# jim-ec/constraint_solver

Hardware: AMD Instinct MI355X
Metric: body·substeps/sec at 262k rigid bodies, 20 substeps/frame; 1/2/4/8 GPU (higher is better)
Workload: dtype f64

## Files before the change

### constraint_solver_amd/csrc/xpbd_contacts.h

```cpp
#pragma once

#include "xpbd_pairs.h"

namespace xpbd {

struct Joint {
    uint32_t body_a, body_b;
    double anchor_a[3], anchor_b[3];
    double distance;
    double axis_a[3], axis_b[3];
    uint32_t kind, reserved;
};

struct JointLimit {
    uint32_t joint, kind;
    double ref_a[3], ref_b[3];
    double lower, upper;
};

struct GridInfo {
    double edge;
    int32_t origin[3];
    uint32_t dims[3];
    uint32_t dense;
// ... 20 lines not shown
    uint32_t *nbr_pair;
    uint32_t *pairs;
    double *rec;
    const double *stat_rec;
    const uint32_t *stat_index;
    ContactManifold *manifolds;
    uint8_t *pair_codes;
    unsigned long long *stats;
    uint32_t *scan_scratch;
    const Joint *joints;
    const uint32_t *joint_off;
    const uint32_t *joint_list;
    const JointLimit *limits;
    const uint32_t *limit_off;
    double max_depenetration_speed;
    const uint2 *filter;
    uint32_t *slot_filter;
    uint32_t filter_jointed;
    const double *friction;
    double ground_friction;
    const double *restitution;
    double ground_restitution;
    double bounce_threshold;
};

struct BodySubset {
    const uint32_t *list = nullptr;
    uint32_t count = 0;
    const uint8_t *skip = nullptr;
    double *export_rows = nullptr;
    const double *import_buf = nullptr;
    const uint32_t *import_rows = nullptr;
};

hipError_t launch_bounds_and_cells(const BodyArrays &b, const PolytopeTables &t, const double *shape_radius,
                                   double dt, double pad, const ContactBuffers &c, hipStream_t stream);
hipError_t launch_build_buckets(const BodyArrays &b, const ContactBuffers &c, hipStream_t stream);
hipError_t launch_neighbour_count(const BodyArrays &b, const ContactBuffers &c, hipStream_t stream);
hipError_t launch_neighbour_fill(const BodyArrays &b, const ContactBuffers &c, hipStream_t stream);

hipError_t launch_integrate_ground(const BodyArrays &b, const ShapeTable &s, double h, const ContactBuffers &c,
                                   uint32_t *last_mask, uint32_t *trace_masks, uint32_t trace_row, hipStream_t stream,
                                   const BodySubset &subset = BodySubset());
hipError_t launch_sat_contact_pairs(const BodyArrays &b, const PolytopeTables &t, const ContactBuffers &c,
                                    uint32_t n_pairs, SatScratch *list, hipStream_t stream, bool dense = false);
hipError_t launch_pair_solve_derive(const BodyArrays &b, double *dyn_out, double h, const ContactBuffers &c,
                                    hipStream_t stream, const BodySubset &subset = BodySubset());

hipError_t launch_pair_solve_integrate_ground(const BodyArrays &b, const ShapeTable &s, double h, const ContactBuffers &c,
                                              double *next_rec, uint32_t *last_mask, uint32_t *trace_masks, uint32_t trace_row,
                                              hipStream_t stream, const BodySubset &subset = BodySubset());

hipError_t launch_restitution(const BodyArrays &b, const double *post, const double *start, const ShapeTable &s, const ContactBuffers &c,
                              const uint32_t *ground_masks, hipStream_t stream);

hipError_t launch_body_frames(const BodyArrays &b, double *rec, hipStream_t stream);
hipError_t launch_stat_records(const BodyArrays &b, double *stat_rec, hipStream_t stream);
hipError_t launch_body_frames_aos(const BodyArrays &b, double *frames, hipStream_t stream);

hipError_t launch_export_dynamic(const BodyArrays &b, const uint32_t *indices, uint32_t n, double *buf, hipStream_t stream);
hipError_t launch_import_dynamic(const BodyArrays &b, const uint32_t *indices, const uint32_t *rows, uint32_t n, const double *buf,
                                 hipStream_t stream);

constexpr uint32_t kMaxEditEntries = 1u << 29;
hipError_t launch_set_wrench(const BodyArrays &b, const uint32_t *indices, uint32_t n, const double *force, const double *torque,
                             hipStream_t stream);
hipError_t launch_apply_impulses(const BodyArrays &b, const xpbd_impulse *list, uint32_t n, hipStream_t stream);

// ... 13 lines not shown
```

### constraint_solver_amd/csrc/xpbd_contacts.hip

```cpp
#include <cfloat>
#include <type_traits>

#include "xpbd_contacts.h"
#include "xpbd_step.hpp"

namespace xpbd {
namespace {

constexpr uint32_t kBlock = 256;
#ifndef XPBD_SMALL_WORLD
#define XPBD_SMALL_WORLD 16384
#endif
constexpr uint32_t kSmallWorld = XPBD_SMALL_WORLD;
#ifndef XPBD_PAIR_SOLVE_MIN_WAVES
#define XPBD_PAIR_SOLVE_MIN_WAVES 2
#endif

__device__ __forceinline__ uint32_t cell_hash(int32_t x, int32_t y, int32_t z)
{
    return ((uint32_t)x * 73856093u) ^ ((uint32_t)y * 19349663u) ^ ((uint32_t)z * 83492791u);
}

__device__ __forceinline__ uint32_t block_scan_exclusive(uint32_t v, uint32_t *total)
{
    __shared__ uint32_t wave_sum[kBlock / 64];
    const uint32_t lane = threadIdx.x & 63u, wave = threadIdx.x >> 6;
    uint32_t inc = v;
#pragma unroll
    for (uint32_t d = 1; d < 64; d <<= 1) {
        const uint32_t up = __shfl_up(inc, d, 64);
        if (lane >= d)
            inc += up;
    }
    if (lane == 63)
        wave_sum[wave] = inc;
    __syncthreads();
    uint32_t before = 0, all = 0;
#pragma unroll
// ... 604 lines not shown
    p.pos = r.pos;
    p.rot = r.rot;
    p.inv_mass = s.inv_mass;
    p.inv_inertia = s.inv_inertia;
    p.com = s.com;
    p.p1 = r.p1;
    p.past = r.past;
    if (past_pos)
        *past_pos = r.past_pos;
    return p;
}

__device__ __forceinline__ Vec3 frame_delta(const Frame &cur, const Frame &past, Vec3 global)
{
    const Vec3 local = inverse(cur) * global;
    return global - past * local;
}

template <class Body>
__device__ __forceinline__ double generalized_inverse_mass(const Body &p, Vec3 point, Vec3 dir)
{
    const Vec3 angular_impulse = conjugate(p.rot) * cross(point - (p.pos + p.com), dir);
    return p.inv_mass + dot(p.inv_inertia * angular_impulse, angular_impulse);
}

#ifndef XPBD_JOINT_LIMIT_INLINE
#define XPBD_JOINT_LIMIT_INLINE __forceinline__
#endif
__device__ XPBD_JOINT_LIMIT_INLINE void joint_limit_terms(const ContactBuffers &c, uint32_t joint, const Joint &jt, bool self_is_a,
                                                          const PairBody &self, const PairBody &other, double compliance, Quat &drot,
                                                          uint32_t &count)
{
    const uint32_t l_end = c.limit_off[joint + 1];
    for (uint32_t l = c.limit_off[joint]; l < l_end; ++l) {
        const JointLimit &lim = c.limits[l];
        const Quat q_a = self_is_a ? self.rot : other.rot, q_b = self_is_a ? other.rot : self.rot;
        const Vec3 a_w = q_a * Vec3{jt.axis_a[0], jt.axis_a[1], jt.axis_a[2]};
        double phi;
        Vec3 n;
        if (lim.kind == XPBD_LIMIT_SWING) {
            const Vec3 b_w = q_b * Vec3{jt.axis_b[0], jt.axis_b[1], jt.axis_b[2]};
            const Vec3 cr = cross(a_w, b_w);
            const double s = length(cr);
            if (s == 0.0)
                continue;
            phi = atan2(s, dot(a_w, b_w));
// ... 12 lines not shown
                p_a = p_a - n * dot(p_a, n);
                p_b = p_b - n * dot(p_b, n);
            }
            phi = atan2(dot(cross(p_a, p_b), n), dot(p_a, p_b));
        }
        const double clamped = phi < lim.lower ? lim.lower : (phi > lim.upper ? lim.upper : phi);
        const double err = phi - clamped;
        if (err == 0.0)
            continue;
        const Vec3 n_self = conjugate(self.rot) * n, n_other = conjugate(other.rot) * n;
        const double w_s = dot(self.inv_inertia * n_self, n_self), w_o = dot(other.inv_inertia * n_other, n_other);
        const double w = self_is_a ? w_s + w_o : w_o + w_s;
        const double lambda = err / (w + compliance);
        const Vec3 turn = self_is_a ? lambda * n : (-lambda) * n;
        const Quat spin = quat_sv(0.0, self.inv_inertia * turn);
        drot = drot + (0.5 * spin) * self.rot;
        ++count;
    }
}

#ifndef XPBD_PAIR_SOLVE_ROUND_POINTS
#define XPBD_PAIR_SOLVE_ROUND_POINTS 2
#endif
template <uint32_t G, bool MATERIALS>
__device__ __forceinline__ BodyDynamic pair_solve_derive_body(const ContactBuffers &c, uint32_t i, double h,
                                                              const PairBody &self, Vec3 self_past_pos, uint32_t sub, uint32_t &touching,
                                                              uint32_t &points, const RecordStage &stage = RecordStage())
{
    static_assert(G == 1 || G == kMaxManifoldPoints, "one lane per body or one lane per manifold point");
    const double compliance = 1e-6 / (h * h);
    const double limit = c.max_depenetration_speed > 0.0 ? c.max_depenetration_speed * h : 0.0;
    const double mu_self = MATERIALS ? c.friction[i] : 0.0;

    Vec3 dpos{0.0, 0.0, 0.0};
    Quat drot{0.0, 0.0, 0.0, 0.0};
    uint32_t count = 0;
    auto neighbour_terms = [&](uint32_t j, const ContactManifold *m, uint32_t n_points, uint32_t feature, uint32_t pt_begin, uint32_t pt_end) {
        if (j > i && pt_begin == 0) {
            ++touching;
            points += n_points;
        }
        const PairBody other = load_pair_body(c, j, nullptr, stage);
        const double mu = MATERIALS ? min_mu(mu_self, c.friction[j]) : 0.0;
        const bool self_is_a = i < j;
        const bool ref_is_a = feature != 1u;
        const bool self_is_inc = self_is_a != ref_is_a;
        const bool face = feature != 2u;
        const Plane ref_plane{Vec3{m->plane[0], m->plane[1], m->plane[2]}, m->plane[3]};
        auto point_term = [&](uint32_t pt, Vec3 &term_pos, Quat &term_rot) {
            const Vec3 p_inc{m->point[pt][0], m->point[pt][1], m->point[pt][2]};
            Vec3 p_ref;
            if (face) {
                const double depth = distance(ref_plane, p_inc);
                p_ref = p_inc - depth * ref_plane.normal;
            } else {
                p_ref = Vec3{m->point[1][0], m->point[1][1], m->point[1][2]};
            }
            const Vec3 p_self = self_is_inc ? p_inc : p_ref, p_other = self_is_inc ? p_ref : p_inc;
            const Vec3 correction = p_ref - p_inc;
            const Vec3 moved_self = frame_delta(self.p1, self.past, p_self), moved_other = frame_delta(other.p1, other.past, p_other);
            const Vec3 delta_rel = self_is_inc ? moved_self - moved_other : moved_other - moved_self;
            const Vec3 delta_tangential = delta_rel - project_on(delta_rel, correction);
            const Vec3 c0 = p_inc;
// ... 70 lines not shown
                    touch |= 1ull << (k0 - k_base + u);
        }
        uint32_t j_next = 0, pair_next = 0;
        if (touch) {
            const uint32_t k = k_base + (uint32_t)__ffsll((long long)touch) - 1u;
            j_next = c.nbr[k], pair_next = c.nbr_pair[k];
        }
        const uint32_t chunk = (G > 1 || few) ? kMaxManifoldPoints : (uint32_t)XPBD_PAIR_SOLVE_ROUND_POINTS;
        uint32_t j_cur = 0, pair_cur = 0, code_cur = 0, n_cur = 0, pt = 0;
        while (touch || pt < n_cur) {
            if (pt == n_cur) {
                j_cur = j_next, pair_cur = pair_next;
                touch &= touch - 1ull;
                if (touch) {
                    const uint32_t k = k_base + (uint32_t)__ffsll((long long)touch) - 1u;
                    j_next = c.nbr[k], pair_next = c.nbr_pair[k];
                }
                code_cur = c.pair_codes[pair_cur];
                n_cur = code_cur & ((1u << kPairCodeFeatureShift) - 1u);
                pt = 0;
            }
            if (n_cur) {
                const uint32_t stop = n_cur - pt > chunk ? pt + chunk : n_cur;
                neighbour_terms(j_cur, c.manifolds + pair_cur, n_cur, code_cur >> kPairCodeFeatureShift, pt, stop);
                pt = stop;
            }
        }
    }

    if (c.joint_off) {
        for (uint32_t k = c.joint_off[i]; k < c.joint_off[i + 1]; ++k) {
            const Joint &jt = c.joints[c.joint_list[k]];
            const bool self_is_a = jt.body_a == i;
            const PairBody other = load_pair_body(c, self_is_a ? jt.body_b : jt.body_a, nullptr, stage);
            const Vec3 anchor_self = self_is_a ? Vec3{jt.anchor_a[0], jt.anchor_a[1], jt.anchor_a[2]} : Vec3{jt.anchor_b[0], jt.anchor_b[1], jt.anchor_b[2]};
            const Vec3 anchor_other = self_is_a ? Vec3{jt.anchor_b[0], jt.anchor_b[1], jt.anchor_b[2]} : Vec3{jt.anchor_a[0], jt.anchor_a[1], jt.anchor_a[2]};
            const Vec3 p_self = Frame{frame_origin(self.pos, self.rot, self.com), self.rot} * anchor_self;
            const Vec3 p_other = Frame{frame_origin(other.pos, other.rot, other.com), other.rot} * anchor_other;
            const Vec3 difference = self_is_a ? p_other - p_self : p_self - p_other;
            const double dist = length(difference);
            if (dist != 0.0) {
                const Vec3 dir = difference * (1.0 / dist);
                const double w = generalized_inverse_mass(self, p_self, dir) + generalized_inverse_mass(other, p_other, dir);
                const double lambda = (dist - jt.distance) / (w + compliance);
                const Vec3 impulse = self_is_a ? lambda * dir : (-lambda) * dir;
                dpos = dpos + impulse * self.inv_mass;
                const Vec3 arm = p_self - (self.pos + self.com);
// ... 41 lines not shown
    for (uint32_t off = 32; off; off >>= 1) {
        touching += __shfl_xor(touching, off, 64);
        points += __shfl_xor(points, off, 64);
    }
    __shared__ uint32_t part[2][kBlock / 64];
    if ((threadIdx.x & 63u) == 0) {
        part[0][threadIdx.x >> 6] = touching;
        part[1][threadIdx.x >> 6] = points;
    }
    __syncthreads();
    if (threadIdx.x == 0) {
        uint32_t t = 0, p = 0;
        for (uint32_t w = 0; w < kBlock / 64; ++w) {
            t += part[0][w];
            p += part[1][w];
        }
        if (t)
            atomicAdd(&stats[0], (unsigned long long)t);
        if (p)
            atomicAdd(&stats[1], (unsigned long long)p);
    }
}

template <uint32_t G, bool MATERIALS>
__global__ void __launch_bounds__(kBlock, XPBD_PAIR_SOLVE_MIN_WAVES) k_pair_solve_derive(BodyArrays b, double *__restrict__ dyn_out, double h,
                                                                                        ContactBuffers c, BodySubset subset)
{
    const uint32_t gid = blockIdx.x * blockDim.x + threadIdx.x, slot = gid / G, sub = gid % G;
    constexpr bool kStage = G == 1 && XPBD_PAIR_SOLVE_STAGE_RECORDS;
    __shared__ double2 stage_words[kStage ? 12 * kBlock : 1];
    RecordStage stage;
    if (kStage && !subset.list)
        stage = stage_records(stage_words, c.rec, blockIdx.x * kBlock, b.n);
    uint32_t touching = 0, points = 0, i;
    if (subset_body(subset, b.n, slot, i)) {
        Vec3 past_pos;
        const PairBody self = load_pair_body(c, i, &past_pos, stage);
        const BodyDynamic d = pair_solve_derive_body<G, MATERIALS>(c, i, h, self, past_pos, sub, touching, points, stage);
        if (sub == 0) {
            store_dynamic(dyn_out, b.stride, i, d);
            if (subset.export_rows)
                store_row(subset.export_rows, slot, d);
        }
    }
    block_add_stats(sub == 0 ? touching : 0u, sub == 0 ? points : 0u, c.stats);
}

template <bool TRACE, uint32_t G, bool MATERIALS>
__global__ void __launch_bounds__(kBlock, XPBD_PAIR_SOLVE_MIN_WAVES) k_pair_solve_integrate_ground(
    BodyArrays b, ShapeTable shapes, double h, ContactBuffers c, BodySubset subset, double *__restrict__ next_rec,
    uint32_t *__restrict__ last_mask, uint32_t *__restrict__ trace_masks, uint32_t trace_row)
{
    extern __shared__ double lds[];
    uint32_t *lds_off = reinterpret_cast<uint32_t *>(lds + 3 * shapes.total_verts);
    for (uint32_t k = threadIdx.x; k < 3 * shapes.total_verts; k += blockDim.x)
        lds[k] = shapes.verts[k];
    for (uint32_t k = threadIdx.x; k <= shapes.n_shapes; k += blockDim.x)
        lds_off[k] = shapes.offsets[k];
    __syncthreads();

    const uint32_t gid = blockIdx.x * blockDim.x + threadIdx.x, slot = gid / G, sub = gid % G;
    constexpr bool kStage = G == 1 && XPBD_PAIR_SOLVE_STAGE_RECORDS;
    __shared__ double2 stage_words[kStage ? 12 * kBlock : 1];
    RecordStage stage;
    if (kStage && !subset.list)
        stage = stage_records(stage_words, c.rec, blockIdx.x * kBlock, b.n);
    uint32_t touching = 0, points = 0, i;
    if (subset_body(subset, b.n, slot, i)) {
        const uint32_t st = b.stride;
        BodyDynamic d;
        BodyStatic s;
        {
            Vec3 past_pos;
            const PairBody self = load_pair_body(c, i, &past_pos, stage);
            d = pair_solve_derive_body<G, MATERIALS>(c, i, h, self, past_pos, sub, touching, points, stage);
            s = static_of(b, i, self.inv_mass, self.inv_inertia, self.com);
        }
        if (subset.export_rows && sub == 0)
            store_row(subset.export_rows, slot, d);
        const uint32_t sid = b.shape_id[i];
        const uint32_t v0 = lds_off[sid];
        const double compliance = 1e-6 / (h * h);
        const SubstepFrames f = integrate_body(d, s, h);
        const uint32_t mask = solve_ground<MATERIALS>(d, s, f, compliance, lds + 3 * v0, lds_off[sid + 1] - v0,
                                                      c.max_depenetration_speed > 0.0 ? c.max_depenetration_speed * h : 0.0,
                                                      MATERIALS ? ground_mu(c, i) : 0.0);
        if (sub == 0) {
            store_record(next_rec, i, f.cur, f.past, d.pos, d.rot, f.past_pos);
            last_mask[i] = mask;
            if (TRACE)
                trace_masks[(size_t)trace_row * st + i] = mask;
        }
    }
    block_add_stats(sub == 0 ? touching : 0u, sub == 0 ? points : 0u, c.stats);
}

struct VelBody {
    Vec3 pos;
// ... 458 lines not shown
    if (trace_masks && c.friction)
        launch(std::true_type{}, std::true_type{});
    else if (trace_masks)
        launch(std::true_type{}, std::false_type{});
    else if (c.friction)
        launch(std::false_type{}, std::true_type{});
    else
        launch(std::false_type{}, std::false_type{});
    return hipGetLastError();
}

hipError_t launch_sat_contact_pairs(const BodyArrays &b, const PolytopeTables &t, const ContactBuffers &c,
                                    uint32_t n_pairs, SatScratch *list, hipStream_t stream, bool dense)
{
    return launch_sat_contacts(b, t, c.rec, c.pairs, n_pairs, c.manifolds, c.pair_codes, list, stream, dense);
}

hipError_t launch_pair_solve_derive(const BodyArrays &b, double *dyn_out, double h, const ContactBuffers &c,
                                    hipStream_t stream, const BodySubset &subset)
{
    const uint32_t items = subset.list ? subset.count : b.n;
    if (items == 0)
        return hipSuccess;
    auto launch = [&](auto lanes, auto materials) {
        constexpr uint32_t G = decltype(lanes)::value;
        hipLaunchKernelGGL((k_pair_solve_derive<G, decltype(materials)::value>), dim3(blocks_for(items * G)), dim3(kBlock), 0, stream, b,
                           dyn_out, h, c, subset);
    };
    using Wide = std::integral_constant<uint32_t, kMaxManifoldPoints>;
    using One = std::integral_constant<uint32_t, 1>;
    const bool small = b.n <= kSmallWorld;
    if (small && c.friction)
        launch(Wide{}, std::true_type{});
    else if (small)
        launch(Wide{}, std::false_type{});
    else if (c.friction)
        launch(One{}, std::true_type{});
    else
        launch(One{}, std::false_type{});
    return hipGetLastError();
}

hipError_t launch_restitution(const BodyArrays &b, const double *post, const double *start, const ShapeTable &s, const ContactBuffers &c,
                              const uint32_t *ground_masks, hipStream_t stream)
{
    if (b.n == 0)
        return hipSuccess;
    if (!c.restitution || post == b.dyn || start == b.dyn)
        return hipErrorInvalidValue;
    const size_t lds_bytes = (size_t)s.total_verts * 3 * sizeof(double) + (size_t)(s.n_shapes + 1) * sizeof(uint32_t);
    hipLaunchKernelGGL(k_restitution, dim3(blocks_for(b.n)), dim3(kBlock), lds_bytes, stream, b, post, start, s, c, ground_masks);
    return hipGetLastError();
}

hipError_t launch_pair_solve_integrate_ground(const BodyArrays &b, const ShapeTable &s, double h, const ContactBuffers &c,
                                              double *next_rec, uint32_t *last_mask, uint32_t *trace_masks, uint32_t trace_row,
                                              hipStream_t stream, const BodySubset &subset)
{
    const uint32_t items = subset.list ? subset.count : b.n;
    if (items == 0)
        return hipSuccess;
    const size_t lds_bytes = (size_t)s.total_verts * 3 * sizeof(double) + (size_t)(s.n_shapes + 1) * sizeof(uint32_t);
    auto launch_form = [&](auto trace, auto lanes, auto materials) {
        constexpr uint32_t G = decltype(lanes)::value;
        hipLaunchKernelGGL((k_pair_solve_integrate_ground<decltype(trace)::value, G, decltype(materials)::value>), dim3(blocks_for(items * G)),
                           dim3(kBlock), lds_bytes, stream, b, s, h, c, subset, next_rec, last_mask, trace_masks, trace_row);
    };
    auto launch = [&](auto trace, auto lanes) {
        if (c.friction)
            launch_form(trace, lanes, std::true_type{});
        else
            launch_form(trace, lanes, std::false_type{});
    };
    using Wide = std::integral_constant<uint32_t, kMaxManifoldPoints>;
    using One = std::integral_constant<uint32_t, 1>;
    const bool small = b.n <= kSmallWorld;
    if (trace_masks && small)
        launch(std::true_type{}, Wide{});
    else if (trace_masks)
        launch(std::true_type{}, One{});
    else if (small)
        launch(std::false_type{}, Wide{});
    else
        launch(std::false_type{}, One{});
    return hipGetLastError();
}

hipError_t launch_body_frames_aos(const BodyArrays &b, double *frames, hipStream_t stream)
{
    if (b.n)
        hipLaunchKernelGGL(k_body_frames_aos, dim3(blocks_for(b.n)), dim3(kBlock), 0, stream, b, frames);
    return hipGetLastError();
}

hipError_t launch_export_dynamic(const BodyArrays &b, const uint32_t *indices, uint32_t n, double *buf, hipStream_t stream)
{
    if (n)
        hipLaunchKernelGGL(k_export_dynamic, dim3(blocks_for(n * kDynFields)), dim3(kBlock), 0, stream, b, indices, n, buf);
    return hipGetLastError();
}

hipError_t launch_import_dynamic(const BodyArrays &b, const uint32_t *indices, const uint32_t *rows, uint32_t n, const double *buf,
                                 hipStream_t stream)
{
    if (n)
        hipLaunchKernelGGL(k_import_dynamic, dim3(blocks_for(n * kDynFields)), dim3(kBlock), 0, stream, b, indices, rows, n, buf);
    return hipGetLastError();
// ... 78 lines not shown
```

### constraint_solver_amd/csrc/xpbd_world.cpp

```cpp
#include <algorithm>
#include <cmath>
#include <cstdio>
#include <cstdlib>
#include <cstring>
#include <exception>
#include <limits>
#include <memory>
#include <utility>
#include <vector>

#include <hip/hip_runtime_api.h>

#include "xpbd_internal.h"
#include "xpbd_kernels.h"
#include "xpbd_math.hpp"
#include "xpbd_contacts.h"
#include "xpbd_gjk.h"
#include "xpbd_pairs.h"
#include "xpbd_query.h"
#include "xpbd_report.h"

namespace {

uint32_t round_up(uint32_t v, uint32_t to) { return (v + to - 1) / to * to; }
// ... 55 lines not shown
    struct BroadphaseTotals {
        uint32_t entries, pairs;
        unsigned long long stats[2];
    };
    BroadphaseTotals *bp_totals = nullptr;
    hipEvent_t bp_event = nullptr;
    bool bp_pending = false;
    DeviceBuffer frame_snapshot;
    bool frame_snapshot_valid = false, frame_snapshot_stepped = false;
    struct Joints {
        uint32_t n = 0, n_limits = 0;
        std::vector<xpbd_joint> host;
        void clear() { *this = Joints{}; }
    } joints;
    DeviceBuffer jt_joints, jt_off, jt_list, jt_limits, jt_limit_off;
    struct Filters {
        bool on = false;
        uint32_t flags = 0;
        void clear() { *this = Filters{}; }
    } filters;
    DeviceBuffer ft_filters, cb_slot_filter;
    struct Materials {
        bool on = false;
        double ground_friction = std::numeric_limits<double>::infinity();
        void clear() { *this = Materials{}; }
    } materials;
    DeviceBuffer mt_friction;
    struct Restitution {
        bool on = false;
        double ground = 0.0, bounce_threshold = 0.0;
        void clear() { *this = Restitution{}; }
    } restitution;
    DeviceBuffer rs_restitution, rs_start;
    DeviceBuffer q_rec, q_partials, q_grid, q_cell_start, q_cell_fill, q_items, q_scan, q_brute, q_rays, q_hits;
    DeviceBuffer ed_indices, ed_values, ed_list;
    DeviceBuffer history;
    uint32_t history_length = 0;
    std::vector<uint8_t> history_stepped;
    size_t history_slot_bytes() const { return ((size_t)xpbd::kDynFields * stride * 8 + (size_t)stride * 4 + 255) / 256 * 256; }
    DeviceBuffer sat_counters, sat_survivors, sat_axis_cache, gjk_axis_cache, cb_pair_codes;
    xpbd::SatScratch sat_scratch{nullptr, nullptr, 0, nullptr, true};
    bool sat_two_pass = false;
    uint32_t sat_schedule = XPBD_SAT_SCHEDULE_AUTO;
    unsigned long long stats_touching_seen = 0, stats_pair_substeps = 0, stats_pair_substeps_seen = 0;
    DeviceBuffer gjk_counters, gjk_pairs_scratch;
    xpbd::GjkScratch gjk_scratch{nullptr, nullptr, 0, nullptr, nullptr};
    bool report_on = false;
    bool report_frame = false;
    bool report_keys_ready = false;
    bool report_ready = false;
    bool report_prev_valid = false;
    uint32_t report_substeps = 0, report_cur = 0;
    uint32_t report_counts[4] = {0, 0, 0, 0};
    uint32_t *rep_host = nullptr;
    DeviceBuffer rep_touch, rep_flag, rep_sel, rep_npts, rep_keys[2], rep_scan, rep_ev_flag, rep_pairs, rep_points, rep_events;
    const uint8_t *rep_map_owned = nullptr;
    const uint32_t *rep_map_ids = nullptr;
    xpbd::ContactBuffers contact_buffers(uint32_t frame_set = 0) const
    {
        xpbd::ContactBuffers c{};
        c.centers = cb_centers.as<double>();
        c.radius = cb_radius.as<double>();
        c.cell = cb_cell.as<int32_t>();
// ... 14 lines not shown
        c.nbr_pair = cb_nbr_pair.as<uint32_t>();
        c.pairs = cb_pairs.as<uint32_t>();
        c.rec = (frame_set ? cb_rec_b : cb_rec).as<double>();
        c.stat_rec = stat_shared ? cb_stat_shape.as<double>() : cb_stat_rec.as<double>();
        c.stat_index = stat_shared ? shape_id.as<uint32_t>() : nullptr;
        c.manifolds = cb_manifolds.as<xpbd::ContactManifold>();
        c.pair_codes = cb_pair_codes.as<uint8_t>();
        c.stats = cb_stats.as<unsigned long long>();
        c.scan_scratch = cb_scan.as<uint32_t>();
        c.joints = joints.n ? jt_joints.as<xpbd::Joint>() : nullptr;
        c.joint_off = joints.n ? jt_off.as<uint32_t>() : nullptr;
        c.joint_list = joints.n ? jt_list.as<uint32_t>() : nullptr;
        c.limits = joints.n_limits ? jt_limits.as<xpbd::JointLimit>() : nullptr;
        c.limit_off = joints.n_limits ? jt_limit_off.as<uint32_t>() : nullptr;
        c.filter = filters.on ? ft_filters.as<uint2>() : nullptr;
        c.slot_filter = filters.on ? cb_slot_filter.as<uint32_t>() : nullptr;
        c.filter_jointed = (filters.flags & XPBD_FILTER_JOINTED) ? 1u : 0u;
        c.max_depenetration_speed = max_depenetration_speed;
        c.friction = materials.on ? mt_friction.as<double>() : nullptr;
        c.ground_friction = materials.ground_friction;
        c.restitution = restitution.on ? rs_restitution.as<double>() : nullptr;
        c.ground_restitution = restitution.ground;
        c.bounce_threshold = restitution.bounce_threshold;
        return c;
    }

    xpbd::BodyArrays arrays() const
    {
        return xpbd::BodyArrays{dyn.as<double>(), stat.as<double>(), shape_id.as<uint32_t>(), stride, n};
    }
    xpbd::ShapeTable shapes() const
    {
        return xpbd::ShapeTable{shape_verts.as<double>(), shape_offsets.as<uint32_t>(), n_shapes, total_verts};
    }

    ~xpbd_world()
    {
        (void)hipSetDevice(device);
        if (stream)
            (void)hipStreamSynchronize(stream);
        if (bp_totals)
            (void)hipHostFree(bp_totals);
        if (bp_event)
            (void)hipEventDestroy(bp_event);
        if (rep_host)
            (void)hipHostFree(rep_host);
// ... 217 lines not shown
        w->stats_touching_seen = stats_now[0];
        w->stats_pair_substeps_seen = w->stats_pair_substeps;
    }
    if (!w->sat_counters.ptr) {
        XPBD_HIP_TRY(w->sat_counters.reserve(2 * xpbd::kSurvivorCounters * 4));
        XPBD_HIP_TRY(hipMemsetAsync(w->sat_counters.ptr, 0, 2 * xpbd::kSurvivorCounters * 4, w->stream));
        w->sat_scratch.calls = 0;
    }
    XPBD_HIP_TRY(w->sat_survivors.reserve((size_t)(w->n_pairs ? w->n_pairs : 1) * 2 * 4));
    XPBD_HIP_TRY(w->sat_axis_cache.reserve((size_t)(w->n_pairs ? w->n_pairs : 1) * 2));
    XPBD_HIP_TRY(hipMemsetAsync(w->sat_axis_cache.ptr, 0, (size_t)(w->n_pairs ? w->n_pairs : 1) * 2, w->stream));
    w->sat_scratch.counters = w->sat_counters.as<uint32_t>();
    w->sat_scratch.survivors = w->sat_survivors.as<uint32_t>();
    w->sat_scratch.axis_cache = w->sat_axis_cache.as<uint16_t>();
    if (w->narrowphase == XPBD_NARROWPHASE_GJK_EPA) {
        XPBD_HIP_TRY(w->gjk_axis_cache.reserve((size_t)(w->n_pairs ? w->n_pairs : 1) * 24));
        XPBD_HIP_TRY(hipMemsetAsync(w->gjk_axis_cache.ptr, 0, (size_t)(w->n_pairs ? w->n_pairs : 1) * 24, w->stream));
    }
    XPBD_HIP_TRY(w->cb_nbr.reserve((size_t)(w->n_entries ? w->n_entries : 1) * 4));
    XPBD_HIP_TRY(w->cb_nbr_pair.reserve((size_t)(w->n_entries ? w->n_entries : 1) * 4));
    XPBD_HIP_TRY(w->cb_pairs.reserve((size_t)(w->n_pairs ? w->n_pairs : 1) * 8));
    XPBD_HIP_TRY(w->cb_manifolds.reserve((size_t)(w->n_pairs ? w->n_pairs : 1) * sizeof(xpbd::ContactManifold)));
    XPBD_HIP_TRY(w->cb_pair_codes.reserve((size_t)(w->n_pairs ? w->n_pairs : 1)));
    c = w->contact_buffers();
    XPBD_HIP_TRY(xpbd::launch_neighbour_fill(b, c, w->stream));
    w->have_neighbours = true;
    return report_frame_begin(w);
}

int build_neighbours(xpbd_world *w, double dt)
{
    if (int rc = build_neighbours_enqueue(w, dt))
        return rc;
    return build_neighbours_collect(w);
}

int narrowphase_contacts(xpbd_world *w, const xpbd::BodyArrays &b, const xpbd::ContactBuffers &c)
{
    if (w->narrowphase == XPBD_NARROWPHASE_GJK_EPA) {
        if (int rc = ensure_gjk_scratch(w, w->n_pairs))
            return rc;
        w->gjk_scratch.axis_cache = w->gjk_axis_cache.as<double>();
        w->gjk_scratch.codes = c.pair_codes;
        XPBD_HIP_TRY(xpbd::launch_gjk_epa_pairs(b, w->tables(), c.rec, c.pairs, w->n_pairs, nullptr, c.manifolds,
                                                w->gjk_scratch, true, &w->sat_scratch, w->stream));
    } else {
        XPBD_HIP_TRY(xpbd::launch_sat_contact_pairs(b, w->tables(), c, w->n_pairs, w->sat_two_pass ? &w->sat_scratch : nullptr,
                                                    w->stream, w->sat_scratch.cache_edge_axes ));
    }
    w->stats_pair_substeps += w->n_pairs;
    if (w->report_frame) {
        XPBD_HIP_TRY(xpbd::launch_report_touch(c.pair_codes, w->rep_touch.as<uint32_t>(), w->n_pairs, w->stream));
        ++w->report_substeps;
        w->report_keys_ready = w->report_ready = false;
    }
    return XPBD_OK;
}

int substep_contacts(xpbd_world *w, double h, uint32_t *trace, uint32_t trace_row)
{
    const xpbd::BodyArrays b = w->arrays();
    const xpbd::ContactBuffers c = w->contact_buffers();
    if (c.restitution) {
        XPBD_HIP_TRY(hipMemcpyAsync(w->rs_start.ptr, b.dyn + (size_t)xpbd::D_VEL * b.stride, (size_t)6 * b.stride * 8, hipMemcpyDeviceToDevice,
                                    w->stream));
    }
    XPBD_HIP_TRY(xpbd::launch_integrate_ground(b, w->shapes(), h, c, w->last_mask.as<uint32_t>(), trace, trace_row, w->stream));
    if (int rc = narrowphase_contacts(w, b, c))
        return rc;
    if (!c.restitution) {
        XPBD_HIP_TRY(xpbd::launch_pair_solve_derive(b, b.dyn, h, c, w->stream));
        return XPBD_OK;
    }
    XPBD_HIP_TRY(xpbd::launch_pair_solve_derive(b, w->dyn_alt.as<double>(), h, c, w->stream));
    XPBD_HIP_TRY(xpbd::launch_restitution(b, w->dyn_alt.as<double>(), w->rs_start.as<double>(), w->shapes(), c, w->last_mask.as<uint32_t>(),
                                          w->stream));
    return XPBD_OK;
}

int step_contacts(xpbd_world *w, double dt, double h, uint32_t substeps, uint32_t *trace)
{
    if (!w->has_topology)
        return set_error(XPBD_E_INVALID, "XPBD_MODE_CONTACTS needs xpbd_world_set_polytopes");
    if (int rc = build_neighbours(w, dt))
        return rc;
    if (substeps == 0)
        return XPBD_OK;
    if (w->restitution.on) {
        for (uint32_t k = 0; k < substeps; ++k)
            if (int rc = substep_contacts(w, h, trace, k))
                return rc;
        return XPBD_OK;
    }
    XPBD_HIP_TRY(xpbd::launch_integrate_ground(w->arrays(), w->shapes(), h, w->contact_buffers(0), w->last_mask.as<uint32_t>(), trace, 0,
                                               w->stream));
    for (uint32_t k = 0; k < substeps; ++k) {
        const xpbd::BodyArrays b = w->arrays();
        const xpbd::ContactBuffers c = w->contact_buffers(k & 1u);
        if (int rc = narrowphase_contacts(w, b, c))
            return rc;
        if (k + 1 < substeps) {
            const xpbd::ContactBuffers next = w->contact_buffers((k + 1u) & 1u);
            XPBD_HIP_TRY(xpbd::launch_pair_solve_integrate_ground(b, w->shapes(), h, c, next.rec, w->last_mask.as<uint32_t>(), trace,
                                                                  k + 1, w->stream));
        } else {
            XPBD_HIP_TRY(xpbd::launch_pair_solve_derive(b, b.dyn, h, c, w->stream));
        }
    }
    return XPBD_OK;
}

}

namespace xpbd {

int halo_frame_begin_enqueue(xpbd_world *w, double dt) noexcept
{
    if (!w || w->mode != XPBD_MODE_CONTACTS || !w->has_topology)
        return set_error(XPBD_E_INVALID, "halo_frame_begin: needs XPBD_MODE_CONTACTS and xpbd_world_set_polytopes");
    if (w->n == 0)
        return XPBD_OK;
    if (int rc = bind_device(w))
// ... 58 lines not shown
    return XPBD_OK;
}

namespace {
int halo_pair_solve(xpbd_world *w, double h, uint32_t k, bool last, const BodySubset &subset)
{
    const BodyArrays b = w->arrays();
    const ContactBuffers c = w->contact_buffers(k & 1u);
    if (last)
        XPBD_HIP_TRY(launch_pair_solve_derive(b, b.dyn, h, c, w->stream, subset));
    else
        XPBD_HIP_TRY(launch_pair_solve_integrate_ground(b, w->shapes(), h, c, w->contact_buffers((k + 1u) & 1u).rec, w->last_mask.as<uint32_t>(),
                                                        nullptr, k + 1, w->stream, subset));
    return XPBD_OK;
}
}

int halo_substep_boundary(xpbd_world *w, double h, uint32_t k, bool last, const HaloLists &l) noexcept
{
    if (w->n == 0)
        return XPBD_OK;
    if (int rc = bind_device(w))
        return rc;
    if (int rc = narrowphase_contacts(w, w->arrays(), w->contact_buffers(k & 1u)))
        return rc;
    BodySubset subset;
    subset.list = l.boundary;
    subset.count = l.n_boundary;
    subset.export_rows = l.send;
    return halo_pair_solve(w, h, k, last, subset);
}

int halo_substep_interior(xpbd_world *w, double h, uint32_t k, bool last, const HaloLists &l) noexcept
{
    if (w->n == 0)
        return XPBD_OK;
    if (int rc = bind_device(w))
        return rc;
    BodySubset subset;
    subset.skip = l.skip;
    return halo_pair_solve(w, h, k, last, subset);
}

int halo_substep_ghosts(xpbd_world *w, double h, uint32_t k, bool last, const HaloLists &l) noexcept
{
    if (w->n == 0 || l.n_ghosts == 0)
        return XPBD_OK;
// ... 1005 lines not shown
    w->filters.flags = flags;
    return XPBD_OK;
} XPBD_ABI_CATCH

int xpbd_world_set_materials(xpbd_world *w, const xpbd_material *materials, uint32_t n, double ground_friction)
try {
    static_assert(sizeof(xpbd_material) == 16, "xpbd_material is {friction, reserved}");
    if (!w)
        return set_error(XPBD_E_INVALID, "xpbd_world_set_materials: NULL world");
    XPBD_TRY(xpbd::check_per_body("xpbd_world_set_materials", "materials", materials, n, w->n));
    if (!(ground_friction >= 0.0))
        return set_error(XPBD_E_INVALID, "xpbd_world_set_materials: ground_friction = %g (must be >= 0, +inf allowed)", ground_friction);
    if (int rc = xpbd::check_materials("xpbd_world_set_materials", materials, n))
        return rc;
    if (int rc = bind_device(w))
        return rc;
    XPBD_HIP_TRY(hipStreamSynchronize(w->stream));
    const double inf = std::numeric_limits<double>::infinity();
    if ((!materials || n == 0) && ground_friction == inf) {
        w->materials.clear();
        return XPBD_OK;
    }
    std::vector<double> friction(std::max(w->n, 1u), inf);
    for (uint32_t i = 0; materials && i < n; ++i)
        friction[i] = materials[i].friction;
    XPBD_TRY(upload_table(w->mt_friction, friction.data(), friction.size() * sizeof(double)));
    w->materials.on = true;
    w->materials.ground_friction = ground_friction;
    return XPBD_OK;
} XPBD_ABI_CATCH

int xpbd_world_set_restitution(xpbd_world *w, const double *restitution, uint32_t n, double ground_restitution, double bounce_threshold)
try {
    if (!w)
        return set_error(XPBD_E_INVALID, "xpbd_world_set_restitution: NULL world");
    XPBD_TRY(xpbd::check_per_body("xpbd_world_set_restitution", "restitution", restitution, n, w->n));
    if (!(ground_restitution >= 0.0 && ground_restitution <= 1.0))
        return set_error(XPBD_E_INVALID, "xpbd_world_set_restitution: ground_restitution = %g (must be in [0, 1])", ground_restitution);
    if (!(bounce_threshold >= 0.0 && bounce_threshold <= std::numeric_limits<double>::max()))
        return set_error(XPBD_E_INVALID, "xpbd_world_set_restitution: bounce_threshold = %g (must be >= 0 and finite)", bounce_threshold);
    bool any = ground_restitution > 0.0;
    for (uint32_t i = 0; restitution && i < n; ++i) {
        if (!(restitution[i] >= 0.0 && restitution[i] <= 1.0))
            return set_error(XPBD_E_INVALID, "xpbd_world_set_restitution: restitution[%u] = %g (must be in [0, 1])", i, restitution[i]);
        any = any || restitution[i] > 0.0;
    }
    if (int rc = bind_device(w))
        return rc;
    XPBD_HIP_TRY(hipStreamSynchronize(w->stream));
    if (!any) {
// ... 693 lines not shown
```

Measured before the change: 16.35 billion.

## Precompute per-contact-point direction and lambda once per pair for large worlds

```diff
diff --git a/constraint_solver_amd/csrc/xpbd_contacts.h b/constraint_solver_amd/csrc/xpbd_contacts.h
--- a/constraint_solver_amd/csrc/xpbd_contacts.h
+++ b/constraint_solver_amd/csrc/xpbd_contacts.h
@@ -66,6 +66,7 @@
     const double *restitution;
     double ground_restitution;
     double bounce_threshold;
+    double *pair_points;
 };
 
 struct BodySubset {
@@ -88,6 +89,9 @@
                                    const BodySubset &subset = BodySubset());
 hipError_t launch_sat_contact_pairs(const BodyArrays &b, const PolytopeTables &t, const ContactBuffers &c,
                                     uint32_t n_pairs, SatScratch *list, hipStream_t stream, bool dense = false);
+hipError_t launch_pair_points(const BodyArrays &b, double h, const ContactBuffers &c, uint32_t n_pairs, hipStream_t stream);
+bool pair_points_wanted(const BodyArrays &b);
+bool pair_points_in_use(const BodyArrays &b, const ContactBuffers &c);
 hipError_t launch_pair_solve_derive(const BodyArrays &b, double *dyn_out, double h, const ContactBuffers &c,
                                     hipStream_t stream, const BodySubset &subset = BodySubset());
 
diff --git a/constraint_solver_amd/csrc/xpbd_contacts.hip b/constraint_solver_amd/csrc/xpbd_contacts.hip
--- a/constraint_solver_amd/csrc/xpbd_contacts.hip
+++ b/constraint_solver_amd/csrc/xpbd_contacts.hip
@@ -14,6 +14,9 @@
 constexpr uint32_t kSmallWorld = XPBD_SMALL_WORLD;
 #ifndef XPBD_PAIR_SOLVE_MIN_WAVES
 #define XPBD_PAIR_SOLVE_MIN_WAVES 2
+#endif
+#ifndef XPBD_PAIR_SOLVE_STORED_MIN_WAVES
+#define XPBD_PAIR_SOLVE_STORED_MIN_WAVES 2
 #endif
 
 __device__ __forceinline__ uint32_t cell_hash(int32_t x, int32_t y, int32_t z)
@@ -664,6 +667,121 @@
 {
     const Vec3 angular_impulse = conjugate(p.rot) * cross(point - (p.pos + p.com), dir);
     return p.inv_mass + dot(p.inv_inertia * angular_impulse, angular_impulse);
+}
+
+struct MassBody {
+    Vec3 pos;
+    Quat rot;
+    double inv_mass;
+    Mat3 inv_inertia;
+    Vec3 com;
+};
+
+__device__ __forceinline__ Vec3 record_frame_delta(const double *__restrict__ rec, uint32_t i, Vec3 global)
+{
+    const double2 *r = reinterpret_cast<const double2 *>(rec + (size_t)i * kRecDoubles);
+    double2 v[7];
+#pragma unroll
+    for (int k = 0; k < 7; ++k)
+        v[k] = r[k];
+    const Frame p1{Vec3{v[0].x, v[0].y, v[1].x}, Quat{v[1].y, v[2].x, v[2].y, v[3].x}};
+    const Frame past{Vec3{v[3].y, v[4].x, v[4].y}, Quat{v[5].x, v[5].y, v[6].x, v[6].y}};
+    return frame_delta(p1, past, global);
+}
+
+__device__ __forceinline__ double record_inverse_mass(const ContactBuffers &c, uint32_t i, Vec3 point, Vec3 dir)
+{
+    const double2 *r = reinterpret_cast<const double2 *>(c.rec + (size_t)i * kRecDoubles);
+    const double2 v7 = r[7], v8 = r[8], v9 = r[9], v10 = r[10];
+    const StatRecord s = load_stat_record(c.stat_rec, c.stat_index ? c.stat_index[i] : i);
+    const MassBody m{Vec3{v7.x, v7.y, v8.x}, Quat{v8.y, v9.x, v9.y, v10.x}, s.inv_mass, s.inv_inertia, s.com};
+    return generalized_inverse_mass(m, point, dir);
+}
+
+#ifndef XPBD_PAIR_POINTS_MIN_WAVES
+#define XPBD_PAIR_POINTS_MIN_WAVES 3
+#endif
+template <bool MATERIALS>
+__global__ void __launch_bounds__(kBlock, XPBD_PAIR_POINTS_MIN_WAVES) k_pair_points(ContactBuffers c, uint32_t n_pairs, double h)
+{
+    static_assert(kBlock == 256 && kMaxManifoldPoints == 8, "an entry of `owner` is pair-in-group | point << 8");
+    __shared__ uint16_t owner[kBlock * kMaxManifoldPoints];
+    __shared__ uint8_t codes[kBlock];
+    __shared__ uint32_t wave_total[kBlock / 64];
+    const uint32_t t = threadIdx.x, first = blockIdx.x * kBlock, lane = t & 63u, wave = t >> 6;
+    const uint32_t code = first + t < n_pairs ? (uint32_t)c.pair_codes[first + t] : 0u;
+    const uint32_t n = min(code & ((1u << kPairCodeFeatureShift) - 1u), kMaxManifoldPoints);
+    codes[t] = (uint8_t)code;
+    uint32_t incl = n;
+    for (uint32_t off = 1; off < 64; off <<= 1) {
+        const uint32_t up = __shfl_up(incl, off, 64);
+        if (lane >= off)
+            incl += up;
+    }
+    if (lane == 63u)
+        wave_total[wave] = incl;
+    __syncthreads();
+    uint32_t start = incl - n, total = 0;
+    for (uint32_t w = 0; w < kBlock / 64; ++w) {
+        if (w < wave)
+            start += wave_total[w];
+        total += wave_total[w];
+    }
+    for (uint32_t pt = 0; pt < n; ++pt)
+        owner[start + pt] = (uint16_t)(t | pt << 8);
+    __syncthreads();
+
+    const double compliance = 1e-6 / (h * h);
+    const double limit = c.max_depenetration_speed > 0.0 ? c.max_depenetration_speed * h : 0.0;
+    for (uint32_t rank = t; rank < total; rank += kBlock) {
+        const uint32_t own = owner[rank], pt = own >> 8, pair = first + (own & 255u);
+        const uint32_t feature = (uint32_t)codes[own & 255u] >> kPairCodeFeatureShift;
+        const uint2 ab = reinterpret_cast<const uint2 *>(c.pairs)[pair];
+        const bool ref_is_a = feature != 1u;
+        const uint32_t inc = ref_is_a ? ab.y : ab.x, ref = ref_is_a ? ab.x : ab.y;
+        const ContactManifold *m = c.manifolds + pair;
+        const Vec3 p_inc{m->point[pt][0], m->point[pt][1], m->point[pt][2]};
+        Vec3 p_ref;
+        if (feature != 2u) {
+            const Plane ref_plane{Vec3{m->plane[0], m->plane[1], m->plane[2]}, m->plane[3]};
+            const double depth = distance(ref_plane, p_inc);
+            p_ref = p_inc - depth * ref_plane.normal;
+        } else {
+            p_ref = Vec3{m->point[1][0], m->point[1][1], m->point[1][2]};
+        }
+        const Vec3 correction = p_ref - p_inc;
+        const Vec3 moved_inc = record_frame_delta(c.rec, inc, p_inc);
+        const Vec3 moved_ref = record_frame_delta(c.rec, ref, p_ref);
+        const Vec3 delta_rel = moved_inc - moved_ref;
+        const Vec3 delta_tangential = delta_rel - project_on(delta_rel, correction);
+        double k = 1.0;
+        if (MATERIALS) {
+            const double mu = min_mu(c.friction[ab.x], c.friction[ab.y]);
+            const double bound = mu * length(correction);
+            const double len_t = length(delta_tangential);
+            if (bound < len_t)
+                k = bound / len_t;
+        }
+        const Vec3 c1 = p_ref - k * delta_tangential;
+        const Vec3 difference = c1 - p_inc;
+        const double dist = length(difference);
+        const Vec3 dir = difference * (1.0 / dist);
+        const double w = record_inverse_mass(c, inc, p_inc, dir) + record_inverse_mass(c, ref, p_ref, dir);
+        double error = dist;
+        if (limit > 0.0) {
+            const double len = length(correction);
+            const double closing = len > 0.0 ? dot(delta_rel, correction) / len : 0.0;
+            double allowed = limit - closing;
+            if (!(allowed > 0.0))
+                allowed = 0.0;
+            if (dist > allowed)
+                error = allowed;
+        }
+        const double lambda = (error - 0.0) / (w + compliance);
+        double2 *out = reinterpret_cast<double2 *>(c.pair_points + ((size_t)pair * kMaxManifoldPoints + pt) * 4);
+        out[0] = double2{dir.x, dir.y};
+        out[1] = double2{dir.z, lambda};
+    }
 }
 
 #ifndef XPBD_JOINT_LIMIT_INLINE
@@ -722,12 +840,13 @@
 #ifndef XPBD_PAIR_SOLVE_ROUND_POINTS
 #define XPBD_PAIR_SOLVE_ROUND_POINTS 2
 #endif
-template <uint32_t G, bool MATERIALS>
+template <uint32_t G, bool MATERIALS, bool STORED>
 __device__ __forceinline__ BodyDynamic pair_solve_derive_body(const ContactBuffers &c, uint32_t i, double h,
                                                               const PairBody &self, Vec3 self_past_pos, uint32_t sub, uint32_t &touching,
                                                               uint32_t &points, const RecordStage &stage = RecordStage())
 {
     static_assert(G == 1 || G == kMaxManifoldPoints, "one lane per body or one lane per manifold point");
+    static_assert(G == 1 || !STORED, "the stored form has one lane per body");
     const double compliance = 1e-6 / (h * h);
     const double limit = c.max_depenetration_speed > 0.0 ? c.max_depenetration_speed * h : 0.0;
     const double mu_self = MATERIALS ? c.friction[i] : 0.0;
@@ -735,10 +854,38 @@
     Vec3 dpos{0.0, 0.0, 0.0};
     Quat drot{0.0, 0.0, 0.0, 0.0};
     uint32_t count = 0;
-    auto neighbour_terms = [&](uint32_t j, const ContactManifold *m, uint32_t n_points, uint32_t feature, uint32_t pt_begin, uint32_t pt_end) {
+    auto neighbour_terms = [&](uint32_t j, uint32_t pair, uint32_t n_points, uint32_t feature, uint32_t pt_begin, uint32_t pt_end) {
+        const ContactManifold *m = c.manifolds + pair;
         if (j > i && pt_begin == 0) {
             ++touching;
             points += n_points;
+        }
+        if constexpr (STORED) {
+            const bool self_is_inc = (i < j) != (feature != 1u);
+            const bool face = feature != 2u;
+            const Plane ref_plane{Vec3{m->plane[0], m->plane[1], m->plane[2]}, m->plane[3]};
+            const double2 *stored = reinterpret_cast<const double2 *>(c.pair_points + (size_t)pair * kMaxManifoldPoints * 4);
+            for (uint32_t pt = pt_begin; pt < pt_end; ++pt) {
+                const double2 s0 = stored[2 * pt], s1 = stored[2 * pt + 1];
+                const Vec3 dir{s0.x, s0.y, s1.x};
+                const double lambda = s1.y;
+                Vec3 p_self{m->point[pt][0], m->point[pt][1], m->point[pt][2]};
+                if (!self_is_inc) {
+                    if (face) {
+                        const double depth = distance(ref_plane, p_self);
+                        p_self = p_self - depth * ref_plane.normal;
+                    } else {
+                        p_self = Vec3{m->point[1][0], m->point[1][1], m->point[1][2]};
+                    }
+                }
+                const Vec3 impulse = self_is_inc ? lambda * dir : (-lambda) * dir;
+                dpos = dpos + impulse * self.inv_mass;
+                const Vec3 arm = p_self - (self.pos + self.com);
+                const Quat spin = quat_sv(0.0, cross(self.inv_inertia * arm, impulse));
+                drot = drot + (0.5 * spin) * self.rot;
+                ++count;
+            }
+            return;
         }
         const PairBody other = load_pair_body(c, j, nullptr, stage);
         const double mu = MATERIALS ? min_mu(mu_self, c.friction[j]) : 0.0;
@@ -855,7 +1002,7 @@
             }
             if (n_cur) {
                 const uint32_t stop = n_cur - pt > chunk ? pt + chunk : n_cur;
-                neighbour_terms(j_cur, c.manifolds + pair_cur, n_cur, code_cur >> kPairCodeFeatureShift, pt, stop);
+                neighbour_terms(j_cur, pair_cur, n_cur, code_cur >> kPairCodeFeatureShift, pt, stop);
                 pt = stop;
             }
         }
@@ -943,8 +1090,8 @@
     }
 }
 
-template <uint32_t G, bool MATERIALS>
-__global__ void __launch_bounds__(kBlock, XPBD_PAIR_SOLVE_MIN_WAVES) k_pair_solve_derive(BodyArrays b, double *__restrict__ dyn_out, double h,
+template <uint32_t G, bool MATERIALS, bool STORED>
+__global__ void __launch_bounds__(kBlock, STORED ? XPBD_PAIR_SOLVE_STORED_MIN_WAVES : XPBD_PAIR_SOLVE_MIN_WAVES) k_pair_solve_derive(BodyArrays b, double *__restrict__ dyn_out, double h,
                                                                                         ContactBuffers c, BodySubset subset)
 {
     const uint32_t gid = blockIdx.x * blockDim.x + threadIdx.x, slot = gid / G, sub = gid % G;
@@ -957,7 +1104,7 @@
     if (subset_body(subset, b.n, slot, i)) {
         Vec3 past_pos;
         const PairBody self = load_pair_body(c, i, &past_pos, stage);
-        const BodyDynamic d = pair_solve_derive_body<G, MATERIALS>(c, i, h, self, past_pos, sub, touching, points, stage);
+        const BodyDynamic d = pair_solve_derive_body<G, MATERIALS, STORED>(c, i, h, self, past_pos, sub, touching, points, stage);
         if (sub == 0) {
             store_dynamic(dyn_out, b.stride, i, d);
             if (subset.export_rows)
@@ -967,8 +1114,8 @@
     block_add_stats(sub == 0 ? touching : 0u, sub == 0 ? points : 0u, c.stats);
 }
 
-template <bool TRACE, uint32_t G, bool MATERIALS>
-__global__ void __launch_bounds__(kBlock, XPBD_PAIR_SOLVE_MIN_WAVES) k_pair_solve_integrate_ground(
+template <bool TRACE, uint32_t G, bool MATERIALS, bool STORED>
+__global__ void __launch_bounds__(kBlock, STORED ? XPBD_PAIR_SOLVE_STORED_MIN_WAVES : XPBD_PAIR_SOLVE_MIN_WAVES) k_pair_solve_integrate_ground(
     BodyArrays b, ShapeTable shapes, double h, ContactBuffers c, BodySubset subset, double *__restrict__ next_rec,
     uint32_t *__restrict__ last_mask, uint32_t *__restrict__ trace_masks, uint32_t trace_row)
 {
@@ -994,7 +1141,7 @@
         {
             Vec3 past_pos;
             const PairBody self = load_pair_body(c, i, &past_pos, stage);
-            d = pair_solve_derive_body<G, MATERIALS>(c, i, h, self, past_pos, sub, touching, points, stage);
+            d = pair_solve_derive_body<G, MATERIALS, STORED>(c, i, h, self, past_pos, sub, touching, points, stage);
             s = static_of(b, i, self.inv_mass, self.inv_inertia, self.com);
         }
         if (subset.export_rows && sub == 0)
@@ -1499,22 +1646,39 @@
     const uint32_t items = subset.list ? subset.count : b.n;
     if (items == 0)
         return hipSuccess;
-    auto launch = [&](auto lanes, auto materials) {
+    auto launch_form = [&](auto lanes, auto materials, auto stored) {
         constexpr uint32_t G = decltype(lanes)::value;
-        hipLaunchKernelGGL((k_pair_solve_derive<G, decltype(materials)::value>), dim3(blocks_for(items * G)), dim3(kBlock), 0, stream, b,
-                           dyn_out, h, c, subset);
+        hipLaunchKernelGGL((k_pair_solve_derive<G, decltype(materials)::value, decltype(stored)::value>), dim3(blocks_for(items * G)),
+                           dim3(kBlock), 0, stream, b, dyn_out, h, c, subset);
+    };
+    auto launch = [&](auto lanes, auto stored) {
+        if (c.friction)
+            launch_form(lanes, std::true_type{}, stored);
+        else
+            launch_form(lanes, std::false_type{}, stored);
     };
     using Wide = std::integral_constant<uint32_t, kMaxManifoldPoints>;
     using One = std::integral_constant<uint32_t, 1>;
-    const bool small = b.n <= kSmallWorld;
-    if (small && c.friction)
-        launch(Wide{}, std::true_type{});
-    else if (small)
+    if (b.n <= kSmallWorld)
         launch(Wide{}, std::false_type{});
-    else if (c.friction)
+    else if (pair_points_in_use(b, c))
         launch(One{}, std::true_type{});
     else
         launch(One{}, std::false_type{});
+    return hipGetLastError();
+}
+
+bool pair_points_wanted(const BodyArrays &b) { return b.n > kSmallWorld; }
+bool pair_points_in_use(const BodyArrays &b, const ContactBuffers &c) { return pair_points_wanted(b) && c.pair_points != nullptr; }
+
+hipError_t launch_pair_points(const BodyArrays &b, double h, const ContactBuffers &c, uint32_t n_pairs, hipStream_t stream)
+{
+    if (!pair_points_in_use(b, c) || n_pairs == 0)
+        return hipSuccess;
+    if (c.friction)
+        hipLaunchKernelGGL(k_pair_points<true>, dim3(blocks_for(n_pairs)), dim3(kBlock), 0, stream, c, n_pairs, h);
+    else
+        hipLaunchKernelGGL(k_pair_points<false>, dim3(blocks_for(n_pairs)), dim3(kBlock), 0, stream, c, n_pairs, h);
     return hipGetLastError();
 }
 
@@ -1538,28 +1702,32 @@
     if (items == 0)
         return hipSuccess;
     const size_t lds_bytes = (size_t)s.total_verts * 3 * sizeof(double) + (size_t)(s.n_shapes + 1) * sizeof(uint32_t);
-    auto launch_form = [&](auto trace, auto lanes, auto materials) {
+    auto launch_form = [&](auto trace, auto lanes, auto materials, auto stored) {
         constexpr uint32_t G = decltype(lanes)::value;
-        hipLaunchKernelGGL((k_pair_solve_integrate_ground<decltype(trace)::value, G, decltype(materials)::value>), dim3(blocks_for(items * G)),
-                           dim3(kBlock), lds_bytes, stream, b, s, h, c, subset, next_rec, last_mask, trace_masks, trace_row);
+        hipLaunchKernelGGL((k_pair_solve_integrate_ground<decltype(trace)::value, G, decltype(materials)::value, decltype(stored)::value>),
+                           dim3(blocks_for(items * G)), dim3(kBlock), lds_bytes, stream, b, s, h, c, subset, next_rec, last_mask, trace_masks,
+                           trace_row);
     };
-    auto launch = [&](auto trace, auto lanes) {
+    auto launch_lanes = [&](auto trace, auto lanes, auto stored) {
         if (c.friction)
-            launch_form(trace, lanes, std::true_type{});
+            launch_form(trace, lanes, std::true_type{}, stored);
         else
-            launch_form(trace, lanes, std::false_type{});
+            launch_form(trace, lanes, std::false_type{}, stored);
     };
     using Wide = std::integral_constant<uint32_t, kMaxManifoldPoints>;
     using One = std::integral_constant<uint32_t, 1>;
-    const bool small = b.n <= kSmallWorld;
-    if (trace_masks && small)
-        launch(std::true_type{}, Wide{});
-    else if (trace_masks)
-        launch(std::true_type{}, One{});
-    else if (small)
-        launch(std::false_type{}, Wide{});
+    auto launch = [&](auto trace) {
+        if (b.n <= kSmallWorld)
+            launch_lanes(trace, Wide{}, std::false_type{});
+        else if (pair_points_in_use(b, c))
+            launch_lanes(trace, One{}, std::true_type{});
+        else
+            launch_lanes(trace, One{}, std::false_type{});
+    };
+    if (trace_masks)
+        launch(std::true_type{});
     else
-        launch(std::false_type{}, One{});
+        launch(std::false_type{});
     return hipGetLastError();
 }
 
diff --git a/constraint_solver_amd/csrc/xpbd_world.cpp b/constraint_solver_amd/csrc/xpbd_world.cpp
--- a/constraint_solver_amd/csrc/xpbd_world.cpp
+++ b/constraint_solver_amd/csrc/xpbd_world.cpp
@@ -101,6 +101,7 @@
     DeviceBuffer ft_filters, cb_slot_filter;
     struct Materials {
         bool on = false;
+        bool negative_zero = false;
         double ground_friction = std::numeric_limits<double>::infinity();
         void clear() { *this = Materials{}; }
     } materials;
@@ -118,6 +119,7 @@
     std::vector<uint8_t> history_stepped;
     size_t history_slot_bytes() const { return ((size_t)xpbd::kDynFields * stride * 8 + (size_t)stride * 4 + 255) / 256 * 256; }
     DeviceBuffer sat_counters, sat_survivors, sat_axis_cache, gjk_axis_cache, cb_pair_codes;
+    DeviceBuffer cb_pair_points;
     xpbd::SatScratch sat_scratch{nullptr, nullptr, 0, nullptr, true};
     bool sat_two_pass = false;
     uint32_t sat_schedule = XPBD_SAT_SCHEDULE_AUTO;
@@ -178,6 +180,7 @@
         c.restitution = restitution.on ? rs_restitution.as<double>() : nullptr;
         c.ground_restitution = restitution.ground;
         c.bounce_threshold = restitution.bounce_threshold;
+        c.pair_points = materials.on && materials.negative_zero ? nullptr : cb_pair_points.as<double>();
         return c;
     }
 
@@ -441,6 +444,8 @@
     XPBD_HIP_TRY(w->cb_pairs.reserve((size_t)(w->n_pairs ? w->n_pairs : 1) * 8));
     XPBD_HIP_TRY(w->cb_manifolds.reserve((size_t)(w->n_pairs ? w->n_pairs : 1) * sizeof(xpbd::ContactManifold)));
     XPBD_HIP_TRY(w->cb_pair_codes.reserve((size_t)(w->n_pairs ? w->n_pairs : 1)));
+    if (xpbd::pair_points_wanted(b))
+        XPBD_HIP_TRY(w->cb_pair_points.reserve((size_t)(w->n_pairs ? w->n_pairs : 1) * xpbd::kMaxManifoldPoints * 4 * sizeof(double)));
     c = w->contact_buffers();
     XPBD_HIP_TRY(xpbd::launch_neighbour_fill(b, c, w->stream));
     w->have_neighbours = true;
@@ -454,7 +459,7 @@
     return build_neighbours_collect(w);
 }
 
-int narrowphase_contacts(xpbd_world *w, const xpbd::BodyArrays &b, const xpbd::ContactBuffers &c)
+int narrowphase_contacts(xpbd_world *w, const xpbd::BodyArrays &b, const xpbd::ContactBuffers &c, double h)
 {
     if (w->narrowphase == XPBD_NARROWPHASE_GJK_EPA) {
         if (int rc = ensure_gjk_scratch(w, w->n_pairs))
@@ -467,6 +472,7 @@
         XPBD_HIP_TRY(xpbd::launch_sat_contact_pairs(b, w->tables(), c, w->n_pairs, w->sat_two_pass ? &w->sat_scratch : nullptr,
                                                     w->stream, w->sat_scratch.cache_edge_axes ));
     }
+    XPBD_HIP_TRY(xpbd::launch_pair_points(b, h, c, w->n_pairs, w->stream));
     w->stats_pair_substeps += w->n_pairs;
     if (w->report_frame) {
         XPBD_HIP_TRY(xpbd::launch_report_touch(c.pair_codes, w->rep_touch.as<uint32_t>(), w->n_pairs, w->stream));
@@ -485,7 +491,7 @@
                                     w->stream));
     }
     XPBD_HIP_TRY(xpbd::launch_integrate_ground(b, w->shapes(), h, c, w->last_mask.as<uint32_t>(), trace, trace_row, w->stream));
-    if (int rc = narrowphase_contacts(w, b, c))
+    if (int rc = narrowphase_contacts(w, b, c, h))
         return rc;
     if (!c.restitution) {
         XPBD_HIP_TRY(xpbd::launch_pair_solve_derive(b, b.dyn, h, c, w->stream));
@@ -516,7 +522,7 @@
     for (uint32_t k = 0; k < substeps; ++k) {
         const xpbd::BodyArrays b = w->arrays();
         const xpbd::ContactBuffers c = w->contact_buffers(k & 1u);
-        if (int rc = narrowphase_contacts(w, b, c))
+        if (int rc = narrowphase_contacts(w, b, c, h))
             return rc;
         if (k + 1 < substeps) {
             const xpbd::ContactBuffers next = w->contact_buffers((k + 1u) & 1u);
@@ -621,7 +627,7 @@
         return XPBD_OK;
     if (int rc = bind_device(w))
         return rc;
-    if (int rc = narrowphase_contacts(w, w->arrays(), w->contact_buffers(k & 1u)))
+    if (int rc = narrowphase_contacts(w, w->arrays(), w->contact_buffers(k & 1u), h))
         return rc;
     BodySubset subset;
     subset.list = l.boundary;
@@ -1673,10 +1679,14 @@
         return XPBD_OK;
     }
     std::vector<double> friction(std::max(w->n, 1u), inf);
-    for (uint32_t i = 0; materials && i < n; ++i)
+    bool negative_zero = false;
+    for (uint32_t i = 0; materials && i < n; ++i) {
         friction[i] = materials[i].friction;
+        negative_zero |= friction[i] == 0.0 && std::signbit(friction[i]);
+    }
     XPBD_TRY(upload_table(w->mt_friction, friction.data(), friction.size() * sizeof(double)));
     w->materials.on = true;
+    w->materials.negative_zero = negative_zero;
     w->materials.ground_friction = ground_friction;
     return XPBD_OK;
 } XPBD_ABI_CATCH
```

Result: no change. 16.38 billion, median of 6 (+0.2%).
